# aaichert/EpipolarConsistency

Measured on AMD Instinct MI355X. Metric: ECC evaluations/sec (N=400, 1024^2 projections), higher is better.
Workload: dtype f32

## Files before the change

epipolarconsistency_amd/_lib.py:

```python
import ctypes as C
import os

_HERE = os.path.dirname(os.path.abspath(__file__))
LIB_PATH = os.environ.get("ECC_HIP_LIB") or os.path.join(_HERE, "libecc_hip.so")

ECC_OK = 0
FILTER_DERIVATIVE, FILTER_RAMP, FILTER_NONE = 0, 1, 2
POST_IDENTITY, POST_SQUARE_ROOT, POST_LOGARITHM = 0, 1, 2
RADON_EXACT, RADON_FMA = 0, 1
SAMPLING_AUTO, SAMPLING_POLYNOMIAL, SAMPLING_PER_SAMPLE, SAMPLING_REFERENCE = 0, 1, 2, 3


class EccError(RuntimeError):
    def __init__(self, code, message):
        super().__init__("libecc_hip error %d: %s" % (code, message))
        self.code = code


class PreprocessConfig(C.Structure):
    _fields_ = [("process", C.c_int32), ("normalize", C.c_int32), ("bias", C.c_double), ("scale", C.c_double),
                ("apply_log", C.c_int32), ("gaussian_sigma", C.c_double), ("half_kernel_width", C.c_int32),
                ("flip_u", C.c_int32), ("flip_v", C.c_int32), ("zero", C.c_int32 * 4), ("feather", C.c_int32 * 4),
                ("n_blanks", C.c_int32), ("blanks", C.c_void_p)]

# ... 100 lines not shown
    "ecc_group_metric_set_projections": (_i, [_vp, _vp, _i]),
    "ecc_group_metric_set_params": (_i, [_vp, _d, _d, _i]),
    "ecc_group_metric_set_sampling": (_i, [_vp, _i]),
    "ecc_group_metric_set_incremental": (_i, [_vp, _i]),
    "ecc_group_metric_get_object_radius": (_i, [_vp, _pd]),
    "ecc_group_metric_evaluate_all": (_i, [_vp, _vp, _pd]),
    "ecc_group_metric_rank_metric": (_i, [_vp, _i, C.POINTER(_vp)]),
    "ecc_exchange_open": (_i, [C.c_char_p, _i, _i, C.POINTER(C.c_void_p)]),
    "ecc_exchange_sum": (_i, [_vp, _d, _pd]),
    "ecc_exchange_close": (_i, [_vp]),
    "ecc_debug_set_poly_tolerance": (_i, [_vp, C.c_float]),
    "ecc_debug_set_small_eval_bound": (_i, [_vp, _i64]),
    "ecc_debug_set_result_polling": (_i, [_i]),
    "ecc_debug_set_quad_copies": (_i, [_vp, _i]),
    "ecc_debug_set_gradient_launch": (_i, [_vp, _i]),
    "ecc_ctx_set_quad_copies": (_i, [_vp, _i]),
    "ecc_debug_small_stamps": (_i, [_vp, _i]),
    "ecc_debug_step_stamps": (_i, [_vp, _vp]),
    "ecc_ctx_enable_timing": (_i, [_vp, _i]),
    "ecc_ctx_last_kernel_ms": (_i, [_vp, _i, _pf]),
}


def lib():
    global _lib
    if _lib is None:
        if not os.path.exists(LIB_PATH):
            raise ImportError(
                "%s is missing: build it with `python -m epipolarconsistency_amd.build` "
                "(hipcc, gfx950). There is no CPU fallback." % LIB_PATH)
# ... 20 lines not shown
```

epipolarconsistency_amd/api.py:

```python
import ctypes as C

import numpy as np

from . import _lib
from ._lib import (FILTER_DERIVATIVE, FILTER_NONE, FILTER_RAMP, POST_IDENTITY, POST_LOGARITHM,
                   POST_SQUARE_ROOT, EccError, check)


def pack_projection_matrices(Ps):
    return _Ps_colmajor(Ps)


def _Ps_colmajor(Ps):
    A = np.asarray(Ps, dtype=np.float64).reshape(-1, 3, 4)
    return np.ascontiguousarray(A.transpose(0, 2, 1)).reshape(-1, 12)


def _is_torch(x):
    return type(x).__module__.startswith("torch")


class Context:

    def __init__(self, device=0, stream=None):
# ... 303 lines not shown
            check(_lib.lib().ecc_metric_set_record_reuse(self._h, int(self._record_reuse)))
        if self._small_eval is not None:
            check(_lib.lib().ecc_metric_set_small_eval(self._h, int(self._small_eval)))
        self._apply_debug()
        if self._Ps is not None:
            self.setProjectionMatrices(self._Ps)
        return self

    def _apply_debug(self):
        if "poly_tolerance" in self._debug:
            check(_lib.lib().ecc_debug_set_poly_tolerance(self._h, float(self._debug["poly_tolerance"])))
        if "small_eval_bound" in self._debug:
            check(_lib.lib().ecc_debug_set_small_eval_bound(self._h, int(self._debug["small_eval_bound"])))
        if "gradient_launch" in self._debug:
            check(_lib.lib().ecc_debug_set_gradient_launch(self._h, int(self._debug["gradient_launch"])))

    def debugSetGradientLaunch(self, on=True):
        self._debug["gradient_launch"] = 1 if on else 0
        if self._h:
            self._apply_debug()
        return self

    def debugSetPolyTolerance(self, tol_bins):
        self._debug["poly_tolerance"] = float(tol_bins)
        if self._h:
            self._apply_debug()
        return self

    def debugSetSmallEvalBound(self, max_pairs):
        self._debug["small_eval_bound"] = int(max_pairs)
# ... 694 lines not shown
```

epipolarconsistency_amd/csrc/ecc_capi.hip:

```cpp
#include "ecc_capi_internal.h"

#include <condition_variable>
#include <mutex>
#include <thread>

#define ECC_EXPORT extern "C" __attribute__((visibility("default")))

namespace {
thread_local std::string g_last_error;
}

extern "C" int ecc_set_error(int code, const char* msg)
{
    g_last_error = msg ? msg : "";
    return code;
}

namespace ecc_internal {

constexpr double ECC_SPIN_SECONDS = 2.0;

double now_seconds()
{
    return std::chrono::duration<double>(std::chrono::steady_clock::now().time_since_epoch()).count();
// ... 161 lines not shown
{
    return ecc_host::object_radius(P, n_u, n_v);
}

ECC_EXPORT int ecc_ctx_create(int device, void* stream, ecc_ctx** out)
{
    if (!out) return fail(ECC_ERR_INVALID_ARGUMENT, "out is null");
    int n = ecc_device_count();
    if (n <= 0) return fail(ECC_ERR_NO_DEVICE, "no HIP device visible; this library has no CPU fallback");
    if (device < 0 || device >= n) return fail(ECC_ERR_INVALID_ARGUMENT, "device index out of range");
    HIP_TRY(hipSetDevice(device));
    ecc_ctx* c = new (std::nothrow) ecc_ctx();
    if (!c) return fail(ECC_ERR_OUT_OF_MEMORY, "host allocation failed");
    c->device = device;
    c->stream = (hipStream_t)stream;
    *out = c;
    return ECC_OK;
}

ECC_EXPORT int ecc_ctx_destroy(ecc_ctx* ctx)
{
    if (!ctx) return ECC_OK;
    (void)hipSetDevice(ctx->device);
    (void)hipStreamSynchronize(ctx->stream);
    if (ctx->trig_d) (void)hipFree(ctx->trig_d);
    if (ctx->ramp_d) (void)hipFree(ctx->ramp_d);
    if (ctx->poly_d) (void)hipFree(ctx->poly_d);
    if (ctx->pre_tables_d) (void)hipFree(ctx->pre_tables_d);
    if (ctx->pre_tables_h) (void)hipHostFree(ctx->pre_tables_h);
    if (ctx->pre_ev) (void)hipEventDestroy(ctx->pre_ev);
    for (float* b : ctx->pre_scratch_d)
        if (b) (void)hipFree(b);
    if (ctx->radon_T_d) (void)hipFree(ctx->radon_T_d);
    if (ctx->linear_scratch_d) (void)hipFree(ctx->linear_scratch_d);
    for (auto& e : ctx->ev)
        if (e) (void)hipEventDestroy(e);
    delete ctx;
    return ECC_OK;
}

ECC_EXPORT int ecc_ctx_synchronize(ecc_ctx* ctx)
{
// ... 48 lines not shown
```

epipolarconsistency_amd/csrc/ecc_capi_internal.h:

```cpp
#ifndef ECC_CAPI_INTERNAL_H
#define ECC_CAPI_INTERNAL_H

#include <hip/hip_runtime.h>

#include <algorithm>
#include <atomic>
#include <chrono>
#include <cmath>
#include <cstdio>
#include <cstdlib>
#include <cstring>
#include <limits>
#include <memory>
#include <new>
#include <string>
#include <vector>

#include "../../include/ecc_hip.h"
#include "ecc_host_geometry.h"
#include "ecc_layout.h"
#include "ecc_view_changes.h"

extern "C" hipError_t ecc_launch_radon(const EccRadonParams* p, int derivative, hipStream_t stream);
extern "C" hipError_t ecc_launch_dtr_border(float* slabs, int64_t slab_stride, int n_img, int n_alpha, int n_t,
                                            int pitch, hipStream_t stream);
extern "C" hipError_t ecc_launch_ramp(float* slabs, int64_t slab_stride, int n_img, int n_alpha, int n_t, int pitch,
                                      const double* h2_d, hipStream_t stream);
extern "C" hipError_t ecc_launch_dtr_import(const float* src, float* slab, int n_alpha, int n_t, int pitch,
                                            hipStream_t stream);
extern "C" hipError_t ecc_launch_dtr_export(const float* slab, float* dst, int n_alpha, int n_t, int pitch,
                                            hipStream_t stream);
extern "C" hipError_t ecc_launch_build_paired(const float* const* slabs_tbl_d, float* paired_d, int64_t paired_stride, int n,
                                              int rows, int pitch, hipStream_t stream);
extern "C" hipError_t ecc_launch_build_quad(const float* const* slabs_tbl_d, float* quads_d, int64_t quad_stride_floats, int n,
                                            int rows, int pitch, hipStream_t stream);
extern "C" hipError_t ecc_launch_k01(const EccPairParams* p, hipStream_t stream);
extern "C" hipError_t ecc_launch_k01_radii(const EccPairParams* p, const float* radii_d, int period, hipStream_t stream);
extern "C" hipError_t ecc_launch_k01_patched(const EccPairParams* p, const EccSmallEval* x, hipStream_t stream);
extern "C" hipError_t ecc_launch_pairs(const EccPairParams* p, hipStream_t stream);
extern "C" int ecc_small_eval_plan(const EccPairParams* p, long long forced_bound, int* wpp, size_t* lds_bytes);
extern "C" hipError_t ecc_launch_small_eval(const EccPairParams* p, const EccSmallEval* x, hipStream_t stream);
extern "C" int ecc_small_poses_plan(const EccPairParams* p, int Q, int* wpp, size_t* lds_bytes);
extern "C" hipError_t ecc_launch_small_poses(const EccPairParams* p, const EccSmallEval* x, const EccSmallPoses* y, hipStream_t stream);
extern "C" hipError_t ecc_launch_preprocess(const EccPreprocessParams* p, hipStream_t stream);
extern "C" size_t ecc_preprocess_lds_bytes(int k);
extern "C" hipError_t ecc_launch_direct_views(const double* Ps_d, int n, EccDirectView* views, int n_u, int n_v,
                                              hipStream_t stream);
extern "C" hipError_t ecc_launch_direct_transpose(const float* src, float* dst, int n, int W, int H, hipStream_t stream);
extern "C" hipError_t ecc_launch_direct_batch(const EccDirectParams* p, double* total, hipStream_t stream);
extern "C" hipError_t ecc_launch_pair_samples(const EccPairSamplesParams* p, hipStream_t stream);
extern "C" hipError_t ecc_launch_sum_pairs(const float* vals, long long count, double* out, void* scratch, hipStream_t stream);
extern "C" hipError_t ecc_launch_sum_pairs_to_host(const float* vals, long long count, double* out, float* values_host, hipStream_t stream);
extern "C" hipError_t ecc_launch_publish_scalar(const double* value_d, double* host_slot_dev, hipStream_t stream);
extern "C" size_t ecc_sum_scratch_bytes();
// ... 34 lines not shown
typedef EccSlab Slab;

struct ecc_ctx {
    int device = 0;
    hipStream_t stream = nullptr;
    bool timing = false;
    int radon_arithmetic = ECC_RADON_EXACT;
    int quad_copies = ECC_QUAD_COPIES_AUTO;
    hipEvent_t ev[6] = {nullptr, nullptr, nullptr, nullptr, nullptr, nullptr};
    bool ev_valid[3] = {false, false, false};
    float* trig_d = nullptr;
    int trig_n_alpha = 0;
    double* ramp_d = nullptr;
    int ramp_n_t = 0;
    EccPolyTables* poly_d = nullptr;
    char* pre_tables_d = nullptr;
    char* pre_tables_h = nullptr;
    size_t pre_tables_cap = 0;
    hipEvent_t pre_ev = nullptr;
    bool pre_ev_recorded = false;
    float* pre_scratch_d[2] = {nullptr, nullptr};
    size_t pre_scratch_cap[2] = {0, 0};
    float* radon_T_d = nullptr;
    size_t radon_T_cap = 0;
    float* linear_scratch_d = nullptr;
    size_t linear_scratch_cap = 0;
};

struct ecc_dtr {
    ecc_ctx* ctx = nullptr;
// ... 171 lines not shown
    ecc_internal::Kept<ecc_internal::RecordKey> rec;
    PinnedArray<int32_t> reuse_h[2];
    hipEvent_t reuse_ev[2] = {nullptr, nullptr};
    bool reuse_ev_used[2] = {false, false};
    uint64_t reuse_gen = 0;
    std::vector<int> scratch_patched;
    std::vector<int> scratch_stale;
    std::vector<int32_t> scratch_patch_of;
    hipStream_t side_stream = nullptr;
    hipEvent_t fork_ev = nullptr, join_ev = nullptr;
    bool quiet = false;
    uint64_t queue_seq = 0, publish_seq = 0, publish_generation = 0;
    int small_eval = 1;
    int64_t small_max_pairs = -1;
    float economise_tol = ECC_POLY_ECONOMISE_TOL_BINS;
    PinnedArray<int32_t> sidx_h;
    PinnedArray<float> svals_h;
    DeviceArray<unsigned> small_ticket_d;
    int64_t small_pending_count = 0;
    int pose_batching = 1;
    PinnedArray<char> pose_h;
    DeviceArray<float> pose_PinvTs_d;
    DeviceArray<float> pose_Cs_d;
    DeviceArray<int32_t> pose_idx_d;
    DeviceArray<EccPairRecord> pose_records_d;
    DeviceArray<float> pose_values_d;
    DeviceArray<double> pose_partial_d;
    DeviceArray<int32_t> pose_lists_d;
    int64_t last_batched_poses = 0;
    int gradient_launch = 0;
// ... 21 lines not shown

void arm_result(ecc_metric* m);
hipError_t wait_result(ecc_metric* m, hipStream_t stream, double* value);
int set_device(const ecc_ctx* ctx);
int ensure_poly_tables(ecc_ctx* ctx);
void decide_quad_copies(ecc_metric* m);
int ensure_e1(ecc_metric* m);
int fill_pair_params(ecc_metric* m, EccPairParams* p, int64_t mode_count, bool need_e1 = true);
int launch_range(ecc_metric* m, int64_t first, int64_t count, float* pair_values_d, float* cost_d, float* K01_d, double* sum_d,
                 bool synchronous = false);
int evaluate_cached(ecc_metric* m, int64_t first, int64_t count, double* sum_d, float** vals_out);

int sum_poses(ecc_metric* m, const float* base_vals_d, int K, int Q, volatile uint64_t* out, double* out_dev, double* sums);
bool pose_keeps_radius(const ecc_metric* m, double base_radius, int c, const int32_t* views, const double* moved_Ps);

inline hipError_t launch_pairs_timed(ecc_ctx* ctx, const EccPairParams* p, const EccSmallEval* x = nullptr)
{
    if (ctx->timing) {
        const hipError_t e = hipEventRecord(ctx->ev[0], ctx->stream);
        if (e != hipSuccess) return e;
    }
    const hipError_t e = x ? ecc_launch_small_eval(p, x, ctx->stream) : ecc_launch_pairs(p, ctx->stream);
    if (e != hipSuccess || !ctx->timing) return e;
    const hipError_t e1 = hipEventRecord(ctx->ev[1], ctx->stream);
    if (e1 == hipSuccess) ctx->ev_valid[0] = true;
    return e1;
}

}

#endif
```

epipolarconsistency_amd/csrc/ecc_evaluate.hip:

```cpp
#include "ecc_capi_internal.h"
#include "ecc_sum_order.h"

#include <iterator>

#define ECC_EXPORT extern "C" __attribute__((visibility("default")))

using namespace ecc_internal;

namespace {

double pose_now() { return std::chrono::duration<double>(std::chrono::steady_clock::now().time_since_epoch()).count(); }

int resolve_sampling(const ecc_metric* m, int64_t count)
{
    if (m->sampling != ECC_SAMPLING_AUTO) return m->sampling;
    return count <= ECC_SAMPLING_AUTO_REFERENCE_PAIRS ? ECC_SAMPLING_REFERENCE : ECC_SAMPLING_POLYNOMIAL;
}

}
namespace ecc_internal {
int fill_pair_params(ecc_metric* m, EccPairParams* p, int64_t mode_count, bool need_e1)
{
    if (m->n_views < 1) return fail(ECC_ERR_INVALID_ARGUMENT, "projection matrices have not been set");
    if (need_e1) {
// ... 222 lines not shown
        if (m->side_stream) (void)hipStreamDestroy(m->side_stream);
        if (m->fork_ev) (void)hipEventDestroy(m->fork_ev);
        if (m->join_ev) (void)hipEventDestroy(m->join_ev);
        m->side_stream = nullptr;
        m->fork_ev = m->join_ev = nullptr;
        return false;
    }
    return true;
}

int launch_skipping(ecc_metric* m, const EccPairParams& p, const std::vector<int>& changed, bool* pairs_launched)
{
    EccPairParams pa = p;
    pa.skip_enabled = 1;
    for (int v : changed) pa.skip_mask[v >> 5] |= 1u << (v & 31);
    HIP_TRY(launch_pairs_timed(m->ctx, &pa));
    *pairs_launched = true;
    ecc_stamp(m, 4);
    return ECC_OK;
}

int launch_reused(ecc_metric* m, const EccPairParams& p, bool synchronous, bool was_quiet, bool* reused, bool* pairs_launched)
{
    ecc_ctx* ctx = m->ctx;
    const int64_t n = m->n_views;
    const double* Pcur = m->Ps_h[m->set_generation & 1].host;
    std::vector<int>& changed = m->scratch_changed;
    changed_views(Pcur, m->rec.Ps.data(), n, &changed);
    if (!m->dev_valid || (int64_t)m->dev_Ps.size() != 12 * n) return ECC_OK;
    std::vector<int>&stale = m->scratch_stale, &patched = m->scratch_patched;
    changed_views(Pcur, m->dev_Ps.data(), n, &stale);
// ... 101 lines not shown
    if (first < 0 || count < 0 || first + count > n_pairs)
        return fail(ECC_ERR_INVALID_ARGUMENT, "pair range outside [0, n(n-1)/2)");
    if (!m->quads_decided && n_pairs >= 32768 && count > 0) decide_quad_copies(m);
    EccPairParams p;
    int rc = fill_pair_params(m, &p, n_pairs, false);
    if (rc) return rc;
    rc = m->records_d.ensure(count > 0 ? count : 1, ctx->stream);
    if (rc) return rc;
    p.first = first;
    p.count = count;
    p.pair_values = pair_values_d;
    p.cost = cost_d;
    p.K01_out = K01_d;
    p.records = m->records_d.ptr;
    m->last_evaluated_pairs = count;
    if (sum_d && sum_d == m->sum_h.dev && pair_values_d) {
        bool taken = false;
        rc = try_small_eval(m, p, nullptr, &taken);
        if (rc) return rc;
        if (taken) return ECC_OK;
    }

    const int mode = p.reference_arithmetic ? ECC_SAMPLING_REFERENCE : (p.poly ? ECC_SAMPLING_POLYNOMIAL : ECC_SAMPLING_PER_SAMPLE);
    const RecordKey key = {mode, p.object_radius_mm, p.dkappa_user, p.economise_tol};
    const bool size_ok = m->record_reuse >= 2 || count > ECC_RECORD_REUSE_MIN_PAIRS;
    m->eager_e1 = !m->record_reuse || !size_ok;
    const bool keep = m->record_reuse && !K01_d && count > 0;
    const bool rec_match = keep && size_ok && m->rec.matches(first, count, (int)n, key);
    m->rec.valid = false;
    bool reused = false, pairs_launched = false;
    ecc_stamp(m, 3);
    m->stamps[4] = m->stamps[5] = 0.0;
    if (rec_match) {
        rc = launch_reused(m, p, synchronous, was_quiet, &reused, &pairs_launched);
        if (rc) return rc;
    }
    if (!reused) {
        rc = launch_k01_with_e1(m, p);
        if (rc) return rc;
        if (keep) m->rec.take(first, count, (int)n, key, m->Ps_h[m->set_generation & 1].host);
    }
    ecc_stamp(m, 5);
    if (!pairs_launched) HIP_TRY(launch_pairs_timed(ctx, &p));
    if (m->stamps[4] == 0.0) ecc_stamp(m, 4);
    if (sum_d) {
        if (count > 0) HIP_TRY(ecc_launch_sum_pairs(pair_values_d, count, sum_d, m->sum_scratch_d.ptr, ctx->stream));
        else if (sum_d == m->sum_h.dev) std::memset(m->sum_h.host, 0, sizeof(double));
        else HIP_TRY(hipMemsetAsync(sum_d, 0, sizeof(double), ctx->stream));
    }
    m->rec.valid = keep;
    ecc_stamp(m, 6);
    return ECC_OK;
}

int evaluate_cached(ecc_metric* m, int64_t first, int64_t count, double* sum_d, float** vals_out)
{
    ecc_mark_busy(m);
    ecc_ctx* ctx = m->ctx;
// ... 374 lines not shown
            for (int k = 0; k < ECC_POLY_DEG + 2; ++k) *o++ = r.cd[v][k];
    }
    return ECC_OK;
}

ECC_EXPORT int ecc_debug_set_poly_tolerance(ecc_metric* m, float tol_bins)
{
    if (!m) return fail(ECC_ERR_INVALID_ARGUMENT, "metric is null");
    if (!(tol_bins >= 0.f) || tol_bins > 1.f) return fail(ECC_ERR_INVALID_ARGUMENT, "tolerance outside [0, 1] bins");
    m->economise_tol = tol_bins;
    m->rec.valid = false;
    m->cache.valid = false;
    return ECC_OK;
}

ECC_EXPORT int ecc_debug_step_stamps(const ecc_metric* m, double* out8)
{
    if (!m || !out8) return fail(ECC_ERR_INVALID_ARGUMENT, "null argument");
    std::memcpy(out8, m->stamps, sizeof(double) * ECC_STEP_STAMPS);
    return ECC_OK;
}

ECC_EXPORT int ecc_debug_set_small_eval_bound(ecc_metric* m, int64_t max_pairs)
{
    if (!m) return fail(ECC_ERR_INVALID_ARGUMENT, "metric is null");
    m->small_max_pairs = max_pairs < 0 ? -1 : max_pairs;
    return ECC_OK;
}

ECC_EXPORT int ecc_debug_small_stamps(unsigned long long* out, int n_blocks)
// ... 7 lines not shown
```

epipolarconsistency_amd/csrc/ecc_layout.h:

```cpp
#ifndef ECC_LAYOUT_H
#define ECC_LAYOUT_H

#include <stdint.h>

#if defined(__HIPCC__)
#include <hip/hip_runtime.h>
__device__ __forceinline__ void ecc_get_ij_device(long long ij, int n, int& i, int& j)
{
    double nn = (double)n - 0.5;
    int r = (int)floor(nn - sqrt(nn * nn - 2.0 * (double)ij));
    r = max(0, min(r, n - 2));
    while (r > 0 && (long long)r * n - (long long)r * (r + 1) / 2 > ij) --r;
    while ((long long)(r + 1) * n - (long long)(r + 1) * (r + 2) / 2 <= ij) ++r;
    i = r;
    j = (int)(ij - ((long long)r * n - (long long)r * (r + 1) / 2)) + r + 1;
}
#endif

static inline int ecc_layout_pitch(int n_t) { return ((n_t + 2) + 31) / 32 * 32; }
static inline int ecc_layout_rows(int n_alpha) { return n_alpha + 2; }
static inline int64_t ecc_layout_floats(int n_alpha, int n_t)
{
    return (int64_t)ecc_layout_rows(n_alpha) * ecc_layout_pitch(n_t);
}
// ... 17 lines not shown
#ifndef ECC_PAIRS_SPLIT_MAX
#define ECC_PAIRS_SPLIT_MAX 4096
#endif
#ifndef ECC_PAIRS_SPLIT4_MAX
#define ECC_PAIRS_SPLIT4_MAX 2048
#endif
#ifndef ECC_PAIRS_SPLIT8_MAX
#define ECC_PAIRS_SPLIT8_MAX 768
#endif
#ifndef ECC_REFIT_FIRST_MAX_PAIRS
#define ECC_REFIT_FIRST_MAX_PAIRS 16384
#endif
#ifndef ECC_BESIDE_ONE_WAVE_MIN_PAIRS
#define ECC_BESIDE_ONE_WAVE_MIN_PAIRS 32768
#endif
#define ECC_POLY_DEG 10
#define ECC_POLY_CHECKS 3
#ifndef ECC_POLY_KAPPA_FIT_MAX
#define ECC_POLY_KAPPA_FIT_MAX 0.98f
#endif
#if defined(__HIPCC__)
__host__ __device__
#endif
inline float ecc_kappa_fit(float kappa_max) { return kappa_max < ECC_POLY_KAPPA_FIT_MAX ? kappa_max : ECC_POLY_KAPPA_FIT_MAX; }

struct EccPairRecord {
    float K0[8];
    float K1[8];
    int iD0, iD1;
    int ci, cj;
// ... 177 lines not shown
```

epipolarconsistency_amd/csrc/ecc_pairs_device.h:

```cpp
#ifndef ECC_PAIRS_DEVICE_H
#define ECC_PAIRS_DEVICE_H

#include <hip/hip_runtime.h>
#include <float.h>
#include <type_traits>

#include "ecc_layout.h"
#include "ecc_sum_order.h"

namespace {

constexpr int PK_THREADS = 256;
constexpr int PK_MAIN_WAVES = 4;
constexpr int PK_MAIN_THREADS = 64 * PK_MAIN_WAVES;

__device__ __forceinline__ void shift_origin_and_normalize(float x, float y, float* Ki)
{
    Ki[2] += x * Ki[0] + y * Ki[1];
    Ki[5] += x * Ki[3] + y * Ki[4];
    float s0 = sqrtf(Ki[0] * Ki[0] + Ki[1] * Ki[1]);
#pragma unroll
    for (int i = 0; i < 6; i++) Ki[i] /= s0;
}

// ... 74 lines not shown
__device__ __forceinline__ bool main_pair_of_wave(long long count, long long& local)
{
    const int wave = threadIdx.x >> 6;
    const long long nblk = (count + PK_MAIN_WAVES - 1) / PK_MAIN_WAVES;
    const long long per_xcd = (nblk + 7) / 8;
    const long long blk = (long long)(blockIdx.x & 7) * per_xcd + (blockIdx.x >> 3);
    if (blk >= nblk) return false;
    local = (long long)wave * nblk + blk;
    return local < count;
}

inline dim3 main_pairs_grid(long long count)
{
    const long long nblk = (count + PK_MAIN_WAVES - 1) / PK_MAIN_WAVES, per_xcd = (nblk + 7) / 8;
    return dim3((unsigned)(per_xcd * 8));
}

template <bool REDUCE>
__device__ __forceinline__ void sincos_quadrant(float kappa, float& s, float& c)
{
    const float pio2_hi = 1.57079637050628662109375f, pio2_lo = -4.37113900018624283e-8f;
    const bool swap = REDUCE && kappa > 0.785398163397448f;
    const float r = swap ? (pio2_hi - kappa) + pio2_lo : kappa;
    const float z = r * r;
    float ps = fmaf(fmaf(-1.958291686605662e-04f, z, 8.332724682986736e-03f), z, -1.66666641831398e-01f);
    float sn = fmaf(ps, r * z, r);
    float pc = fmaf(fmaf(fmaf(2.445712743792683e-05f, z, -1.3887537643313408e-03f), z, 4.166664928197861e-02f), z, -0.5f);
    float cs = fmaf(pc, z, 1.0f);
    s = swap ? cs : sn;
    c = swap ? sn : cs;
// ... 1051 lines not shown
```

epipolarconsistency_amd/csrc/pairs_kernel.hip:

```cpp
#include <hip/hip_runtime.h>
#include <float.h>

#include "ecc_layout.h"
#include "ecc_pairs_device.h"

namespace {



template <int LANES>
__device__ __forceinline__ void k01_block(const EccPairParams& p, K01Shared<LANES>& sh, EccSmallEvalArg small, bool poison,
                                          const float* radii = nullptr, int radii_period = 1)
{
    constexpr int K01_PAIRS = 64 / LANES;
    k01_fit_block<LANES>(p, (long long)blockIdx.x * K01_PAIRS, K01_PAIRS, sh, small, nullptr, true, radii, radii_period);
    const long long first_pair = (long long)blockIdx.x * K01_PAIRS;
    const long long n_here = min((long long)K01_PAIRS, p.count - first_pair);
    if (n_here > 0) {
        constexpr int RW = (int)(sizeof(EccPairRecord) / 8);
        const int words = (int)n_here * RW;
        if (poison) {
            if (threadIdx.x < n_here) sh.recs[threadIdx.x].K0[6] = __builtin_nanf("");
            __syncthreads();
        }
// ... 24 lines not shown
    k01_block<LANES>(p, sh, nullptr, false, radii, period);
}

template <int LANES>
__global__ __launch_bounds__(256) void k01_patched_kernel(EccPairParams p, EccSmallEval x)
{
    __shared__ K01Shared<LANES> sh;
    typedef const char __attribute__((address_space(4))) * KernargBytes;
    static_assert(alignof(EccSmallEval) == 8 && alignof(EccPairParams) == 8, "layout of the kernel arguments");
    const EccSmallEvalArg xs = (EccSmallEvalArg)((KernargBytes)__builtin_amdgcn_kernarg_segment_ptr() + ((sizeof(EccPairParams) + 7) & ~(size_t)7));
    const bool args_ok = xs->magic == ECC_SMALL_MAGIC && x.magic == ECC_SMALL_MAGIC && xs->patch_count == x.patch_count;
    k01_block<LANES>(p, sh, xs, !args_ok);
}

#ifndef PK_OCCUPANCY
#define PK_OCCUPANCY __attribute__((amdgpu_num_sgpr(96), amdgpu_num_vgpr(36)))
#endif
template <bool DERIV, bool CORR>
__global__ __launch_bounds__(PK_MAIN_THREADS) PK_OCCUPANCY void pairs_kernel(EccPairParams p)
{
    const int lane = threadIdx.x & 63;
    long long local;
    if (!main_pair_of_wave(p.count, local)) return;
    local = uniform_index(local);
    const long long rec_index = p.record_slots ? (long long)__builtin_amdgcn_readfirstlane(p.record_slots[local]) : local;
    const EccPairRecord* __restrict__ rec = p.records + rec_index;
    const int iD0 = __builtin_amdgcn_readfirstlane(rec->iD0), iD1 = __builtin_amdgcn_readfirstlane(rec->iD1);
    if (p.skip_enabled) {
        const unsigned m0 = p.skip_mask[(iD0 >> 5) & (ECC_SKIP_WORDS - 1)], m1 = p.skip_mask[(iD1 >> 5) & (ECC_SKIP_WORDS - 1)];
        if (((m0 >> (iD0 & 31)) | (m1 >> (iD1 & 31))) & 1u) return;
    }
    const int ci = __builtin_amdgcn_readfirstlane(rec->ci), cj = __builtin_amdgcn_readfirstlane(rec->cj);
    double acc = 0.0;
    double mom2 = 0.0, mom3 = 0.0, mom4 = 0.0;
    pair_accumulate<DERIV, CORR>(p, rec, iD0, iD1, lane, acc, mom2, mom3, mom4);
    wave_sum_pair<CORR>(acc, mom2, mom3, mom4);
    const float val = pair_value<CORR>(acc, mom2, mom3, mom4);
    if (lane == 0) store_pair_value(p, local, ci, cj, val);
}

template <bool DERIV, int WPP>
__global__ __launch_bounds__(WPP > 4 ? 64 * WPP : PK_THREADS) void pairs_split_kernel(EccPairParams p, int stage_stride)
{
    constexpr int PPW = WPP > 4 ? 1 : 4 / WPP;
    extern __shared__ float stage_all[];
    const int lane = threadIdx.x & 63, wave = threadIdx.x >> 6;
    const int slot = wave / WPP, sub = wave % WPP;
    long long local = (long long)blockIdx.x * PPW + slot;
    const bool live = local < p.count;
    local = uniform_index(local);
    double acc = 0.0, m2 = 0.0, m3 = 0.0, m4 = 0.0;
    const EccPairRecord* __restrict__ rec = nullptr;
    float* stage = stage_all + (size_t)slot * stage_stride;
// ... 202 lines not shown
    return hipGetLastError();
}

extern "C" hipError_t ecc_launch_k01_patched(const EccPairParams* p, const EccSmallEval* x, hipStream_t stream)
{
    if (p->count <= 0) return hipSuccess;
    if (p->count > ECC_K01_WIDE_MAX_PAIRS || p->patch_count || x->patch_count < 0 || x->patch_count > ECC_SMALL_PATCH_MAX) return hipErrorInvalidValue;
    EccSmallEval xx = *x;
    xx.magic = ECC_SMALL_MAGIC;
    k01_launch_form(p->count, [&](auto LANES, dim3 grid) {
        if constexpr (decltype(LANES)::value > 1) hipLaunchKernelGGL(k01_patched_kernel<decltype(LANES)::value>, grid, dim3(256), 0, stream, *p, xx);
    });
    return hipGetLastError();
}

extern "C" hipError_t ecc_launch_pairs(const EccPairParams* p, hipStream_t stream)
{
    if (p->count <= 0) return hipSuccess;
    const long long nblk = (p->count + 3) / 4;
    if (p->reference_arithmetic) {
        const int stride = (p->k_limit + 63) & ~63;
        const size_t wide_lds = sizeof(float) * (size_t)stride * (p->use_corr ? 3u : 1u);
        if (p->reference_split > 1 && p->count <= ECC_REFERENCE_WIDE_MAX_PAIRS && wide_lds <= 48 * 1024) {
            const dim3 grid((unsigned)p->count), block(ECC_REFERENCE_WIDE_THREADS);
            if (p->use_corr) hipLaunchKernelGGL((pairs_reference_wide_kernel<true>), grid, block, wide_lds, stream, *p, stride);
            else hipLaunchKernelGGL((pairs_reference_wide_kernel<false>), grid, block, wide_lds, stream, *p, stride);
        } else if (p->reference_split > 1) {
            if (p->use_corr) hipLaunchKernelGGL((pairs_reference_kernel<true, 4>), dim3((unsigned)p->count), dim3(PK_THREADS), 0, stream, *p);
            else hipLaunchKernelGGL((pairs_reference_kernel<false, 4>), dim3((unsigned)p->count), dim3(PK_THREADS), 0, stream, *p);
        } else {
            if (p->use_corr) hipLaunchKernelGGL((pairs_reference_kernel<true, 1>), dim3((unsigned)nblk), dim3(PK_THREADS), 0, stream, *p);
            else hipLaunchKernelGGL((pairs_reference_kernel<false, 1>), dim3((unsigned)nblk), dim3(PK_THREADS), 0, stream, *p);
        }
        return hipGetLastError();
    }
    if (!p->use_corr && !p->skip_enabled && p->beside_another_launch < 2 && p->count <= ECC_PAIRS_SPLIT_MAX) {
        const int wpp = (p->count <= ECC_PAIRS_SPLIT8_MAX && !p->beside_another_launch) ? 8 : (p->count <= ECC_PAIRS_SPLIT4_MAX ? 4 : 2);
        const int ppw = wpp > 4 ? 1 : 4 / wpp;
        const int stride = (p->k_limit + 63) & ~63;
        const size_t lds = sizeof(float) * (size_t)ppw * (size_t)stride;
        if (lds <= 48 * 1024) {
            const dim3 grid((unsigned)((p->count + ppw - 1) / ppw)), block(wpp > 4 ? 64 * wpp : PK_THREADS);
            if (p->is_derivative) {
                if (wpp == 8) hipLaunchKernelGGL((pairs_split_kernel<true, 8>), grid, block, lds, stream, *p, stride);
                else if (wpp == 4) hipLaunchKernelGGL((pairs_split_kernel<true, 4>), grid, block, lds, stream, *p, stride);
                else hipLaunchKernelGGL((pairs_split_kernel<true, 2>), grid, block, lds, stream, *p, stride);
            } else {
                if (wpp == 8) hipLaunchKernelGGL((pairs_split_kernel<false, 8>), grid, block, lds, stream, *p, stride);
                else if (wpp == 4) hipLaunchKernelGGL((pairs_split_kernel<false, 4>), grid, block, lds, stream, *p, stride);
                else hipLaunchKernelGGL((pairs_split_kernel<false, 2>), grid, block, lds, stream, *p, stride);
            }
            return hipGetLastError();
        }
    }
    const dim3 grid = main_pairs_grid(p->count), block(PK_MAIN_THREADS);
    if (p->use_corr) {
        if (p->is_derivative)
            hipLaunchKernelGGL((pairs_kernel<true, true>), grid, block, 0, stream, *p);
        else
            hipLaunchKernelGGL((pairs_kernel<false, true>), grid, block, 0, stream, *p);
    } else {
        if (p->is_derivative)
            hipLaunchKernelGGL((pairs_kernel<true, false>), grid, block, 0, stream, *p);
        else
            hipLaunchKernelGGL((pairs_kernel<false, false>), grid, block, 0, stream, *p);
    }
    return hipGetLastError();
}
```

include/ecc_hip.h:

```cpp
#ifndef ECC_HIP_H
#define ECC_HIP_H

#include <stdint.h>

#ifdef __cplusplus
extern "C" {
#endif

#define ECC_HIP_VERSION 100

enum {
    ECC_OK = 0,
    ECC_ERR_INVALID_ARGUMENT = 1,
    ECC_ERR_HIP = 2,
    ECC_ERR_OUT_OF_MEMORY = 3,
    ECC_ERR_NO_DEVICE = 4,
    ECC_ERR_UNSUPPORTED = 5
};

enum { ECC_FILTER_DERIVATIVE = 0, ECC_FILTER_RAMP = 1, ECC_FILTER_NONE = 2 };
enum { ECC_POST_IDENTITY = 0, ECC_POST_SQUARE_ROOT = 1, ECC_POST_LOGARITHM = 2 };

typedef struct ecc_ctx ecc_ctx;
typedef struct ecc_dtr ecc_dtr;
// ... 191 lines not shown
#define ECC_EXCHANGE_MAX_RANKS 64
typedef struct ecc_exchange ecc_exchange;
int ecc_exchange_open(const char* name, int rank, int world, ecc_exchange** out);
int ecc_exchange_sum(ecc_exchange* ex, double partial, double* total);
int ecc_exchange_close(ecc_exchange* ex);

int ecc_ctx_enable_timing(ecc_ctx* ctx, int enable);
int ecc_ctx_last_kernel_ms(ecc_ctx* ctx, int which, float* ms);

#define ECC_POLY_ECONOMISE_TOL_BINS 2e-8f
int ecc_debug_set_poly_tolerance(ecc_metric* m, float tol_bins);
int ecc_debug_set_small_eval_bound(ecc_metric* m, int64_t max_pairs);
int ecc_debug_set_result_polling(int on);
int ecc_debug_set_quad_copies(ecc_ctx* ctx, int on);
int ecc_debug_set_gradient_launch(ecc_metric* m, int on);
#define ECC_QUAD_COPIES_AUTO (-1)
#define ECC_QUAD_COPIES_OFF 0
#define ECC_QUAD_COPIES_ON 1
int ecc_ctx_set_quad_copies(ecc_ctx* ctx, int mode);
int ecc_metric_device_bytes(const ecc_metric* m, int64_t* paired_bytes, int64_t* quad_bytes, int64_t* other_bytes);
int ecc_debug_small_stamps(unsigned long long* out, int n_blocks);
#define ECC_STEP_STAMPS 8
int ecc_debug_step_stamps(const ecc_metric* m, double* out8);

#ifdef __cplusplus
}
#endif
#endif
```

Before: 3200.

## Add persistent work-queue schedule for the pairs kernel behind a debug switch

Adds an atomic per-XCD ticket queue so that a capped grid of persistent workgroups can pull several pairs per wave, and makes it selectable through a new debug setter. The default schedule (-1) keeps the classic launch path, but the main pairs kernel is rewritten anyway: it reads kernel arguments from the kernarg segment, moves the wave reduction into a noinline epilogue, and pins occupancy at 7 waves per EU. The intent is to cut wave launch and tail overhead. The cost is extra atomics, a device allocation per context, and possible register or occupancy changes on the default path.

```diff
diff --git a/epipolarconsistency_amd/_lib.py b/epipolarconsistency_amd/_lib.py
--- a/epipolarconsistency_amd/_lib.py
+++ b/epipolarconsistency_amd/_lib.py
@@ -138,6 +138,7 @@
     "ecc_debug_set_result_polling": (_i, [_i]),
     "ecc_debug_set_quad_copies": (_i, [_vp, _i]),
     "ecc_debug_set_gradient_launch": (_i, [_vp, _i]),
+    "ecc_debug_set_pair_schedule": (_i, [_vp, _i, _i, _i]),
     "ecc_ctx_set_quad_copies": (_i, [_vp, _i]),
     "ecc_debug_small_stamps": (_i, [_vp, _i]),
     "ecc_debug_step_stamps": (_i, [_vp, _vp]),
diff --git a/epipolarconsistency_amd/api.py b/epipolarconsistency_amd/api.py
--- a/epipolarconsistency_amd/api.py
+++ b/epipolarconsistency_amd/api.py
@@ -341,6 +341,14 @@
             check(_lib.lib().ecc_debug_set_small_eval_bound(self._h, int(self._debug["small_eval_bound"])))
         if "gradient_launch" in self._debug:
             check(_lib.lib().ecc_debug_set_gradient_launch(self._h, int(self._debug["gradient_launch"])))
+        if "pair_schedule" in self._debug:
+            check(_lib.lib().ecc_debug_set_pair_schedule(self._h, *self._debug["pair_schedule"]))
+
+    def debugSetPairSchedule(self, mode=-1, pairs_per_wave=None, max_workgroups=0):
+        self._debug["pair_schedule"] = (int(mode), -1 if pairs_per_wave is None else int(pairs_per_wave), int(max_workgroups))
+        if self._h:
+            self._apply_debug()
+        return self
 
     def debugSetGradientLaunch(self, on=True):
         self._debug["gradient_launch"] = 1 if on else 0
diff --git a/epipolarconsistency_amd/csrc/ecc_capi.hip b/epipolarconsistency_amd/csrc/ecc_capi.hip
--- a/epipolarconsistency_amd/csrc/ecc_capi.hip
+++ b/epipolarconsistency_amd/csrc/ecc_capi.hip
@@ -199,6 +199,14 @@
     if (!c) return fail(ECC_ERR_OUT_OF_MEMORY, "host allocation failed");
     c->device = device;
     c->stream = (hipStream_t)stream;
+    const size_t queue_bytes = sizeof(unsigned) * 2 * ECC_PAIR_QUEUE_SET_WORDS;
+    if (hipMalloc((void**)&c->pair_queue_d, queue_bytes) != hipSuccess || hipMemset(c->pair_queue_d, 0, queue_bytes) != hipSuccess ||
+        hipStreamSynchronize(nullptr) != hipSuccess) {
+        (void)hipGetLastError();
+        if (c->pair_queue_d) (void)hipFree(c->pair_queue_d);
+        delete c;
+        return fail(ECC_ERR_OUT_OF_MEMORY, "device allocation of the pair queue failed");
+    }
     *out = c;
     return ECC_OK;
 }
@@ -211,6 +219,7 @@
     if (ctx->trig_d) (void)hipFree(ctx->trig_d);
     if (ctx->ramp_d) (void)hipFree(ctx->ramp_d);
     if (ctx->poly_d) (void)hipFree(ctx->poly_d);
+    if (ctx->pair_queue_d) (void)hipFree(ctx->pair_queue_d);
     if (ctx->pre_tables_d) (void)hipFree(ctx->pre_tables_d);
     if (ctx->pre_tables_h) (void)hipHostFree(ctx->pre_tables_h);
     if (ctx->pre_ev) (void)hipEventDestroy(ctx->pre_ev);
diff --git a/epipolarconsistency_amd/csrc/ecc_capi_internal.h b/epipolarconsistency_amd/csrc/ecc_capi_internal.h
--- a/epipolarconsistency_amd/csrc/ecc_capi_internal.h
+++ b/epipolarconsistency_amd/csrc/ecc_capi_internal.h
@@ -38,6 +38,7 @@
 extern "C" hipError_t ecc_launch_k01_radii(const EccPairParams* p, const float* radii_d, int period, hipStream_t stream);
 extern "C" hipError_t ecc_launch_k01_patched(const EccPairParams* p, const EccSmallEval* x, hipStream_t stream);
 extern "C" hipError_t ecc_launch_pairs(const EccPairParams* p, hipStream_t stream);
+extern "C" hipError_t ecc_launch_pairs_queued(const EccPairParams* p, const EccPairQueue* q, int max_workgroups, hipStream_t stream);
 extern "C" int ecc_small_eval_plan(const EccPairParams* p, long long forced_bound, int* wpp, size_t* lds_bytes);
 extern "C" hipError_t ecc_launch_small_eval(const EccPairParams* p, const EccSmallEval* x, hipStream_t stream);
 extern "C" int ecc_small_poses_plan(const EccPairParams* p, int Q, int* wpp, size_t* lds_bytes);
@@ -102,6 +103,8 @@
     double* ramp_d = nullptr;
     int ramp_n_t = 0;
     EccPolyTables* poly_d = nullptr;
+    unsigned* pair_queue_d = nullptr;
+    uint64_t pair_queue_launches = 0;
     char* pre_tables_d = nullptr;
     char* pre_tables_h = nullptr;
     size_t pre_tables_cap = 0;
@@ -303,6 +306,9 @@
     int small_eval = 1;
     int64_t small_max_pairs = -1;
     float economise_tol = ECC_POLY_ECONOMISE_TOL_BINS;
+    int pair_schedule = -1;
+    int pair_queue_pairs_per_wave = ECC_PAIR_QUEUE_PAIRS_PER_WAVE;
+    int pair_queue_max_workgroups = 0;
     PinnedArray<int32_t> sidx_h;
     PinnedArray<float> svals_h;
     DeviceArray<unsigned> small_ticket_d;
@@ -354,13 +360,30 @@
 int sum_poses(ecc_metric* m, const float* base_vals_d, int K, int Q, volatile uint64_t* out, double* out_dev, double* sums);
 bool pose_keeps_radius(const ecc_metric* m, double base_radius, int c, const int32_t* views, const double* moved_Ps);
 
-inline hipError_t launch_pairs_timed(ecc_ctx* ctx, const EccPairParams* p, const EccSmallEval* x = nullptr)
+inline bool pair_launch_queued(const ecc_metric* m, const EccPairParams* p, hipStream_t stream)
+{
+    if (!m || m->pair_schedule == 0 || !m->ctx->pair_queue_d || stream != m->ctx->stream) return false;
+    if (p->indices || p->record_slots || p->value_slots || p->cost || p->K01_out || p->reference_arithmetic || p->count <= 0) return false;
+    return m->pair_schedule == 1;
+}
+
+inline hipError_t launch_pairs_timed(ecc_ctx* ctx, const EccPairParams* p, const EccSmallEval* x = nullptr, const ecc_metric* m = nullptr)
 {
     if (ctx->timing) {
         const hipError_t e = hipEventRecord(ctx->ev[0], ctx->stream);
         if (e != hipSuccess) return e;
     }
-    const hipError_t e = x ? ecc_launch_small_eval(p, x, ctx->stream) : ecc_launch_pairs(p, ctx->stream);
+    hipError_t e;
+    if (x) {
+        e = ecc_launch_small_eval(p, x, ctx->stream);
+    } else if (pair_launch_queued(m, p, ctx->stream)) {
+        const uint64_t k = ctx->pair_queue_launches++;
+        const EccPairQueue q = {ctx->pair_queue_d + (k & 1) * ECC_PAIR_QUEUE_SET_WORDS, ctx->pair_queue_d + ((k + 1) & 1) * ECC_PAIR_QUEUE_SET_WORDS,
+                                m->pair_queue_pairs_per_wave};
+        e = ecc_launch_pairs_queued(p, &q, m->pair_queue_max_workgroups, ctx->stream);
+    } else {
+        e = ecc_launch_pairs(p, ctx->stream);
+    }
     if (e != hipSuccess || !ctx->timing) return e;
     const hipError_t e1 = hipEventRecord(ctx->ev[1], ctx->stream);
     if (e1 == hipSuccess) ctx->ev_valid[0] = true;
diff --git a/epipolarconsistency_amd/csrc/ecc_evaluate.hip b/epipolarconsistency_amd/csrc/ecc_evaluate.hip
--- a/epipolarconsistency_amd/csrc/ecc_evaluate.hip
+++ b/epipolarconsistency_amd/csrc/ecc_evaluate.hip
@@ -260,7 +260,7 @@
     EccPairParams pa = p;
     pa.skip_enabled = 1;
     for (int v : changed) pa.skip_mask[v >> 5] |= 1u << (v & 31);
-    HIP_TRY(launch_pairs_timed(m->ctx, &pa));
+    HIP_TRY(launch_pairs_timed(m->ctx, &pa, nullptr, m));
     *pairs_launched = true;
     ecc_stamp(m, 4);
     return ECC_OK;
@@ -392,7 +392,7 @@
     p.K01_out = K01_d;
     p.records = m->records_d.ptr;
     m->last_evaluated_pairs = count;
-    if (sum_d && sum_d == m->sum_h.dev && pair_values_d) {
+    if (sum_d && sum_d == m->sum_h.dev && pair_values_d && m->pair_schedule != 1) {
         bool taken = false;
         rc = try_small_eval(m, p, nullptr, &taken);
         if (rc) return rc;
@@ -419,7 +419,7 @@
         if (keep) m->rec.take(first, count, (int)n, key, m->Ps_h[m->set_generation & 1].host);
     }
     ecc_stamp(m, 5);
-    if (!pairs_launched) HIP_TRY(launch_pairs_timed(ctx, &p));
+    if (!pairs_launched) HIP_TRY(launch_pairs_timed(ctx, &p, nullptr, m));
     if (m->stamps[4] == 0.0) ecc_stamp(m, 4);
     if (sum_d) {
         if (count > 0) HIP_TRY(ecc_launch_sum_pairs(pair_values_d, count, sum_d, m->sum_scratch_d.ptr, ctx->stream));
@@ -824,6 +824,17 @@
     return ECC_OK;
 }
 
+ECC_EXPORT int ecc_debug_set_pair_schedule(ecc_metric* m, int mode, int pairs_per_wave, int max_workgroups)
+{
+    if (!m) return fail(ECC_ERR_INVALID_ARGUMENT, "metric is null");
+    if (mode < -1 || mode > 1) return fail(ECC_ERR_INVALID_ARGUMENT, "pair schedule must be -1 (auto), 0 (classic) or 1 (queue)");
+    if (max_workgroups < 0) return fail(ECC_ERR_INVALID_ARGUMENT, "the grid cap must not be negative");
+    m->pair_schedule = mode;
+    m->pair_queue_pairs_per_wave = pairs_per_wave < 0 ? ECC_PAIR_QUEUE_PAIRS_PER_WAVE : pairs_per_wave;
+    m->pair_queue_max_workgroups = max_workgroups;
+    return ECC_OK;
+}
+
 ECC_EXPORT int ecc_debug_step_stamps(const ecc_metric* m, double* out8)
 {
     if (!m || !out8) return fail(ECC_ERR_INVALID_ARGUMENT, "null argument");
diff --git a/epipolarconsistency_amd/csrc/ecc_layout.h b/epipolarconsistency_amd/csrc/ecc_layout.h
--- a/epipolarconsistency_amd/csrc/ecc_layout.h
+++ b/epipolarconsistency_amd/csrc/ecc_layout.h
@@ -55,6 +55,18 @@
 #ifndef ECC_BESIDE_ONE_WAVE_MIN_PAIRS
 #define ECC_BESIDE_ONE_WAVE_MIN_PAIRS 32768
 #endif
+#define ECC_PAIR_QUEUE_HEADS 32
+#define ECC_PAIR_QUEUE_HEAD_WORDS 32
+#define ECC_PAIR_QUEUE_SET_WORDS (ECC_PAIR_QUEUE_HEADS * ECC_PAIR_QUEUE_HEAD_WORDS)
+#ifndef ECC_PAIR_QUEUE_PAIRS_PER_WAVE
+#define ECC_PAIR_QUEUE_PAIRS_PER_WAVE 4
+#endif
+struct EccPairQueue {
+    unsigned* heads;
+    unsigned* spent;
+    int pairs_per_wave;
+};
+
 #define ECC_POLY_DEG 10
 #define ECC_POLY_CHECKS 3
 #ifndef ECC_POLY_KAPPA_FIT_MAX
diff --git a/epipolarconsistency_amd/csrc/ecc_pairs_device.h b/epipolarconsistency_amd/csrc/ecc_pairs_device.h
--- a/epipolarconsistency_amd/csrc/ecc_pairs_device.h
+++ b/epipolarconsistency_amd/csrc/ecc_pairs_device.h
@@ -112,6 +112,33 @@
 {
     const long long nblk = (count + PK_MAIN_WAVES - 1) / PK_MAIN_WAVES, per_xcd = (nblk + 7) / 8;
     return dim3((unsigned)(per_xcd * 8));
+}
+
+__device__ __forceinline__ unsigned queue_request(unsigned* heads, int label, int wave, int lane)
+{
+    unsigned t = 0;
+    if (lane == 0)
+        t = __hip_atomic_fetch_add(heads + (label * PK_MAIN_WAVES + wave) * ECC_PAIR_QUEUE_HEAD_WORDS, 1u, __ATOMIC_RELAXED, __HIP_MEMORY_SCOPE_AGENT);
+    return t;
+}
+
+__device__ __forceinline__ bool queue_ticket_pair(unsigned t, int label, int wave, long long count, long long& local)
+{
+    const long long nblk = (count + PK_MAIN_WAVES - 1) / PK_MAIN_WAVES;
+    const long long per_xcd = (nblk + 7) / 8;
+    const long long blk = (long long)label * per_xcd + t;
+    local = (long long)wave * nblk + blk;
+    return (long long)t < per_xcd && blk < nblk && local < count;
+}
+
+__device__ __forceinline__ bool queue_take(unsigned* heads, int& label, int& tried, int wave, int lane, long long count, long long& local, int& ticket)
+{
+#pragma nounroll
+    for (; tried < 8; ++tried, label = (label + 1) & 7) {
+        ticket = __builtin_amdgcn_readfirstlane((int)queue_request(heads, label, wave, lane));
+        if (queue_ticket_pair((unsigned)ticket, label, wave, count, local)) return true;
+    }
+    return false;
 }
 
 template <bool REDUCE>
diff --git a/epipolarconsistency_amd/csrc/pairs_kernel.hip b/epipolarconsistency_amd/csrc/pairs_kernel.hip
--- a/epipolarconsistency_amd/csrc/pairs_kernel.hip
+++ b/epipolarconsistency_amd/csrc/pairs_kernel.hip
@@ -62,29 +62,100 @@
 }
 
 #ifndef PK_OCCUPANCY
-#define PK_OCCUPANCY __attribute__((amdgpu_num_sgpr(96), amdgpu_num_vgpr(36)))
+#define PK_OCCUPANCY __attribute__((amdgpu_num_sgpr(96), amdgpu_num_vgpr(36), amdgpu_waves_per_eu(7, 7)))
 #endif
+struct PairsKernelArgs {
+    EccPairParams p;
+    EccPairQueue q;
+};
+typedef const PairsKernelArgs __attribute__((address_space(4))) * PairsKernelArgsPtr;
+typedef const EccPairRecord __attribute__((address_space(4))) * ConstantRecords;
+
+__device__ __forceinline__ int lane_of_wave()
+{
+    int l;
+    asm volatile("v_mbcnt_lo_u32_b32 %0, -1, 0\n\tv_mbcnt_hi_u32_b32 %0, -1, %0" : "=v"(l));
+    return l;
+}
+
+template <bool CORR>
+__device__ __attribute__((noinline)) float pair_epilogue(double acc, double mom2, double mom3, double mom4)
+{
+    wave_sum_pair<CORR>(acc, mom2, mom3, mom4);
+    return pair_value<CORR>(acc, mom2, mom3, mom4);
+}
+
+constexpr int PK_QUEUE_LEFT_SHIFT = 9, PK_QUEUE_LEFT_MAX = (1 << 21) - 1;
+
 template <bool DERIV, bool CORR>
-__global__ __launch_bounds__(PK_MAIN_THREADS) PK_OCCUPANCY void pairs_kernel(EccPairParams p)
-{
-    const int lane = threadIdx.x & 63;
-    long long local;
-    if (!main_pair_of_wave(p.count, local)) return;
-    local = uniform_index(local);
-    const long long rec_index = p.record_slots ? (long long)__builtin_amdgcn_readfirstlane(p.record_slots[local]) : local;
-    const EccPairRecord* __restrict__ rec = p.records + rec_index;
-    const int iD0 = __builtin_amdgcn_readfirstlane(rec->iD0), iD1 = __builtin_amdgcn_readfirstlane(rec->iD1);
-    if (p.skip_enabled) {
-        const unsigned m0 = p.skip_mask[(iD0 >> 5) & (ECC_SKIP_WORDS - 1)], m1 = p.skip_mask[(iD1 >> 5) & (ECC_SKIP_WORDS - 1)];
-        if (((m0 >> (iD0 & 31)) | (m1 >> (iD1 & 31))) & 1u) return;
-    }
-    const int ci = __builtin_amdgcn_readfirstlane(rec->ci), cj = __builtin_amdgcn_readfirstlane(rec->cj);
-    double acc = 0.0;
-    double mom2 = 0.0, mom3 = 0.0, mom4 = 0.0;
-    pair_accumulate<DERIV, CORR>(p, rec, iD0, iD1, lane, acc, mom2, mom3, mom4);
-    wave_sum_pair<CORR>(acc, mom2, mom3, mom4);
-    const float val = pair_value<CORR>(acc, mom2, mom3, mom4);
-    if (lane == 0) store_pair_value(p, local, ci, cj, val);
+__global__ __launch_bounds__(PK_MAIN_THREADS) PK_OCCUPANCY void pairs_kernel(EccPairParams p, EccPairQueue q)
+{
+    static_assert(alignof(EccPairParams) == 8 && alignof(EccPairQueue) == 8 && offsetof(PairsKernelArgs, q) == ((sizeof(EccPairParams) + 7) & ~(size_t)7),
+                  "layout of the kernel arguments");
+    int state, t_cur;
+    {
+        long long local;
+        const int wave = __builtin_amdgcn_readfirstlane((int)(threadIdx.x >> 6));
+        int label = (int)(blockIdx.x & 7), tried = 0, left = 1;
+        if (!q.heads) {
+            t_cur = (int)(blockIdx.x >> 3);
+            if (!queue_ticket_pair((unsigned)t_cur, label, wave, p.count, local)) return;
+        } else {
+            if (blockIdx.x == 0 && threadIdx.x < ECC_PAIR_QUEUE_HEADS) q.spent[threadIdx.x * ECC_PAIR_QUEUE_HEAD_WORDS] = 0u;
+            if (!queue_take(q.heads, label, tried, wave, (int)(threadIdx.x & 63), p.count, local, t_cur)) return;
+            left = q.pairs_per_wave > 0 && q.pairs_per_wave < PK_QUEUE_LEFT_MAX ? q.pairs_per_wave : PK_QUEUE_LEFT_MAX;
+        }
+        state = label | (tried << 3) | (wave << 7) | (left << PK_QUEUE_LEFT_SHIFT);
+    }
+    PairsKernelArgsPtr ka = (PairsKernelArgsPtr)__builtin_amdgcn_kernarg_segment_ptr();
+    for (;;) {
+        asm volatile("" : "+s"(ka));
+        int t_next;
+        {
+            const EccPairParams& pt = ((const PairsKernelArgs*)ka)->p;
+            const int lane = lane_of_wave();
+            long long local;
+            queue_ticket_pair((unsigned)t_cur, state & 7, (state >> 7) & 3, pt.count, local);
+            local = uniform_index(local);
+            unsigned ticket = 0;
+            if ((state >> PK_QUEUE_LEFT_SHIFT) > 1) ticket = queue_request(((const PairsKernelArgs*)ka)->q.heads, state & 7, (state >> 7) & 3, lane);
+            const long long rec_index = pt.record_slots ? (long long)__builtin_amdgcn_readfirstlane(pt.record_slots[local]) : local;
+            const EccPairRecord* __restrict__ rec = (const EccPairRecord*)((ConstantRecords)pt.records + rec_index);
+            const int iD0 = __builtin_amdgcn_readfirstlane(rec->iD0), iD1 = __builtin_amdgcn_readfirstlane(rec->iD1);
+            bool skip = false;
+            if (pt.skip_enabled) {
+                const unsigned m0 = pt.skip_mask[(iD0 >> 5) & (ECC_SKIP_WORDS - 1)], m1 = pt.skip_mask[(iD1 >> 5) & (ECC_SKIP_WORDS - 1)];
+                skip = (((m0 >> (iD0 & 31)) | (m1 >> (iD1 & 31))) & 1u) != 0;
+            }
+            t_next = __builtin_amdgcn_readfirstlane((int)ticket);
+            asm volatile("" : "+s"(t_next), "+s"(state), "+s"(t_cur));
+            if (!skip) {
+                double acc = 0.0;
+                double mom2 = 0.0, mom3 = 0.0, mom4 = 0.0;
+                pair_accumulate<DERIV, CORR>(pt, rec, iD0, iD1, lane, acc, mom2, mom3, mom4);
+                const float val = pair_epilogue<CORR>(acc, mom2, mom3, mom4);
+                asm volatile("" : "+s"(ka));
+                const EccPairParams& ps = ((const PairsKernelArgs*)ka)->p;
+                long long at;
+                queue_ticket_pair((unsigned)t_cur, state & 7, (state >> 7) & 3, ps.count, at);
+                at = uniform_index(at);
+                if (lane_of_wave() == 0) {
+                    const EccPairRecord* rs = (const EccPairRecord*)((ConstantRecords)ps.records + (ps.record_slots ? (long long)__builtin_amdgcn_readfirstlane(ps.record_slots[at]) : at));
+                    store_pair_value(ps, at, rs->ci, rs->cj, val);
+                }
+            }
+        }
+        if ((state >> PK_QUEUE_LEFT_SHIFT) <= 1) return;
+        state -= 1 << PK_QUEUE_LEFT_SHIFT;
+        asm volatile("" : "+s"(ka));
+        const long long count = ((const PairsKernelArgs*)ka)->p.count;
+        long long local;
+        t_cur = t_next;
+        if (queue_ticket_pair((unsigned)t_cur, state & 7, (state >> 7) & 3, count, local)) continue;
+        int label = (state + 1) & 7, tried = ((state >> 3) & 15) + 1;
+        if (!queue_take(((const PairsKernelArgs*)ka)->q.heads, label, tried, (state >> 7) & 3, lane_of_wave(), count, local, t_cur)) return;
+        state = label | (tried << 3) | (state & ~127);
+    }
 }
 
 template <bool DERIV, int WPP>
@@ -317,9 +388,11 @@
     return hipGetLastError();
 }
 
-extern "C" hipError_t ecc_launch_pairs(const EccPairParams* p, hipStream_t stream)
+extern "C" hipError_t ecc_launch_pairs_queued(const EccPairParams* p, const EccPairQueue* q, int max_workgroups, hipStream_t stream)
 {
     if (p->count <= 0) return hipSuccess;
+    if (q && q->heads && (p->reference_arithmetic || p->record_slots || !q->spent)) return hipErrorInvalidValue;
+    const bool queued = q && q->heads;
     const long long nblk = (p->count + 3) / 4;
     if (p->reference_arithmetic) {
         const int stride = (p->k_limit + 63) & ~63;
@@ -337,7 +410,7 @@
         }
         return hipGetLastError();
     }
-    if (!p->use_corr && !p->skip_enabled && p->beside_another_launch < 2 && p->count <= ECC_PAIRS_SPLIT_MAX) {
+    if (!queued && !p->use_corr && !p->skip_enabled && p->beside_another_launch < 2 && p->count <= ECC_PAIRS_SPLIT_MAX) {
         const int wpp = (p->count <= ECC_PAIRS_SPLIT8_MAX && !p->beside_another_launch) ? 8 : (p->count <= ECC_PAIRS_SPLIT4_MAX ? 4 : 2);
         const int ppw = wpp > 4 ? 1 : 4 / wpp;
         const int stride = (p->k_limit + 63) & ~63;
@@ -356,17 +429,40 @@
             return hipGetLastError();
         }
     }
-    const dim3 grid = main_pairs_grid(p->count), block(PK_MAIN_THREADS);
+    dim3 grid = main_pairs_grid(p->count);
+    const dim3 block(PK_MAIN_THREADS);
+    EccPairQueue qq = {nullptr, nullptr, 1};
+    if (queued) {
+        qq = *q;
+        const long long r = qq.pairs_per_wave > 0 ? qq.pairs_per_wave : 0;
+        long long wgs = (nblk + r - 1) / (r > 0 ? r : 1);
+        if (r == 0) {
+            int dev = 0, cus = 0;
+            if (hipGetDevice(&dev) != hipSuccess || hipDeviceGetAttribute(&cus, hipDeviceAttributeMultiprocessorCount, dev) != hipSuccess)
+                return hipGetLastError();
+            wgs = 7LL * cus;
+        }
+        if (wgs > (long long)grid.x) wgs = grid.x;
+        wgs = (wgs + 7) / 8 * 8;
+        if (max_workgroups > 0 && wgs > max_workgroups) wgs = max_workgroups;
+        if (r > 0 && wgs * r < nblk) qq.pairs_per_wave = 0;
+        grid = dim3((unsigned)wgs);
+    }
     if (p->use_corr) {
         if (p->is_derivative)
-            hipLaunchKernelGGL((pairs_kernel<true, true>), grid, block, 0, stream, *p);
+            hipLaunchKernelGGL((pairs_kernel<true, true>), grid, block, 0, stream, *p, qq);
         else
-            hipLaunchKernelGGL((pairs_kernel<false, true>), grid, block, 0, stream, *p);
+            hipLaunchKernelGGL((pairs_kernel<false, true>), grid, block, 0, stream, *p, qq);
     } else {
         if (p->is_derivative)
-            hipLaunchKernelGGL((pairs_kernel<true, false>), grid, block, 0, stream, *p);
+            hipLaunchKernelGGL((pairs_kernel<true, false>), grid, block, 0, stream, *p, qq);
         else
-            hipLaunchKernelGGL((pairs_kernel<false, false>), grid, block, 0, stream, *p);
-    }
-    return hipGetLastError();
-}
+            hipLaunchKernelGGL((pairs_kernel<false, false>), grid, block, 0, stream, *p, qq);
+    }
+    return hipGetLastError();
+}
+
+extern "C" hipError_t ecc_launch_pairs(const EccPairParams* p, hipStream_t stream)
+{
+    return ecc_launch_pairs_queued(p, nullptr, 0, stream);
+}
diff --git a/include/ecc_hip.h b/include/ecc_hip.h
--- a/include/ecc_hip.h
+++ b/include/ecc_hip.h
@@ -229,6 +229,7 @@
 int ecc_debug_set_result_polling(int on);
 int ecc_debug_set_quad_copies(ecc_ctx* ctx, int on);
 int ecc_debug_set_gradient_launch(ecc_metric* m, int on);
+int ecc_debug_set_pair_schedule(ecc_metric* m, int mode, int pairs_per_wave, int max_workgroups);
 #define ECC_QUAD_COPIES_AUTO (-1)
 #define ECC_QUAD_COPIES_OFF 0
 #define ECC_QUAD_COPIES_ON 1
```

Result: slower. 1901 (-40.6%).
